# kyleliang919/distributed-lion-pytorch

Hardware: AMD Instinct MI355X
Metric: tokens/sec + all-reduce bytes/step, GPT-2 CLM at 1/2/4/8 MI355X (higher is better)
Workload: dtype bf16; 1 GPU; model=gpt2 (124.4M params), trainable_params=124439808, base_weights=bf16, global_batch=160, task=clm, gradient_checkpointing=False, micro_batch=20, grad_accum=8, seq_len=1024, parallelism=dp1, optimizer=distributed Lion (majority vote), lr 0.0001, wd 0.1, exchange=a2a, impl=native

## Files before the change

distributed_lion_pytorch_amd/csrc/bindings.cpp:

```cpp
#include <ATen/ATen.h>
#include <c10/core/DeviceGuard.h>
#include <c10/hip/HIPStream.h>
#include <torch/library.h>

#include <hip/hip_runtime.h>

#include <cmath>
#include <cstdlib>
#include <string>
#include <tuple>
#include <vector>

#include "kernels.h"

namespace dlion {
enum class Layout : int { NT = 0, NN = 1, TN = 2, TT = 3 };
bool lt_gemm(const void* a, int64_t lda, const void* b, int64_t ldb, void* c, int64_t ldc, const void* bias,
             int64_t M, int64_t N, int64_t K, int epi, int device, hipStream_t s, Layout lay, bool accumulate);
}

namespace {

using at::Tensor;

// ... 981 lines not shown
    check_bf16_contig(*dwte, "dwte");
    TORCH_CHECK(dwte->dim() == 2 && dwte->size(1) == C, "dlion embed: dwte must be [V, C]");
    TORCH_CHECK(sid.has_value() && perm.has_value() && sid->numel() == n && perm->numel() == n &&
                    sid->scalar_type() == at::kLong && perm->scalar_type() == at::kLong && sid->is_contiguous() &&
                    perm->is_contiguous(),
                "dlion embed: the token gradient needs sorted ids and their permutation (int64 [n])");
    V = dwte->size(0);
  }
  if (dwpe.has_value()) {
    check_bf16_contig(*dwpe, "dwpe");
    TORCH_CHECK(dwpe->size(-1) == C && dwpe->size(0) >= T, "dlion embed: dwpe must be [>= T, C]");
  }
  const c10::DeviceGuard g(dx.device());
  const auto dp = drop_params(p);
  check_hip(dlion::launch_embed_bwd(dx.data_ptr(), dwte.has_value() ? sid->data_ptr<int64_t>() : nullptr,
                                    dwte.has_value() ? perm->data_ptr<int64_t>() : nullptr,
                                    dwte.has_value() ? dwte->data_ptr() : nullptr,
                                    dwpe.has_value() ? dwpe->data_ptr() : nullptr, n, static_cast<int>(C),
                                    static_cast<int>(T), V, pos_accumulate ? 1 : 0, static_cast<uint32_t>(seed),
                                    dp.first, dp.second, cur_stream()),
            "embed_bwd");
}

void scale_acc_(const Tensor& x, const Tensor& s, const Tensor& y, bool accumulate) {
  check_bf16_contig(x, "x");
  check_bf16_contig(y, "y");
  check_dev(s, "s");
  TORCH_CHECK(s.scalar_type() == at::kFloat && s.numel() >= 1, "dlion scale_acc: s must be float32");
  TORCH_CHECK(x.numel() == y.numel() && x.numel() % 8 == 0, "dlion scale_acc: size mismatch / numel % 8 != 0");
  const c10::DeviceGuard g(x.device());
  check_hip(dlion::launch_scale_acc(x.data_ptr(), s.data_ptr<float>(), y.data_ptr(), x.numel(), accumulate ? 1 : 0,
                                    cur_stream()),
            "scale_acc");
}

Tensor gemm_nt_stamped(const Tensor& a, const Tensor& b, const Tensor& stamps) {
  check_gemm_operand(a, "a");
  check_gemm_operand(b, "b");
  TORCH_CHECK(gemm_nt_supported(a, b), "dlion gemm: unsupported shape");
  const int64_t blocks = ((a.size(0) + 255) / 256) * ((b.size(0) + 255) / 256);
  TORCH_CHECK(stamps.is_cuda() && stamps.scalar_type() == at::kLong && stamps.is_contiguous() &&
                  stamps.numel() >= blocks * 8,
              "dlion gemm: stamps must be int64 [blocks, 8]");
  auto c = at::empty({a.size(0), b.size(0)}, a.options());
  const c10::DeviceGuard g(a.device());
  check_hip(dlion::launch_gemm_nt_stamped(a.data_ptr(), static_cast<int>(a.stride(0)), b.data_ptr(),
                                          static_cast<int>(b.stride(0)), c.data_ptr(), static_cast<int>(c.stride(0)),
                                          static_cast<int>(a.size(0)), static_cast<int>(b.size(0)),
                                          static_cast<int>(a.size(1)),
                                          reinterpret_cast<unsigned long long*>(stamps.data_ptr<int64_t>()),
                                          cur_stream()),
            "gemm_nt_stamped");
  return c;
}

std::tuple<Tensor, Tensor> gemm_nt_gelu_d(const Tensor& a, const Tensor& b, const Tensor& bias, bool exact) {
  auto h = at::empty({a.size(0), b.size(0)}, a.options());
  auto d = at::empty({a.size(0), b.size(0)}, a.options());
  gemm_nt_launch(a, b, h, &bias, &d, exact ? 7 : 6);
  return {h, d};
}

std::tuple<Tensor, Tensor> gemm_nt_dmul(const Tensor& a, const Tensor& b, const Tensor& d) {
  auto dz = at::empty({a.size(0), b.size(0)}, a.options());
  auto part = at::empty({2 * ((a.size(0) + 255) / 256), b.size(0)}, a.options().dtype(at::kFloat));
  gemm_nt_launch(a, b, dz, nullptr, &d, 8, &part);
// ... 358 lines not shown
  Tensor part = check_skinny("skinny_gemm_w4", x, N, bias, out, splits, per);
  const int64_t M = x.size(0);
  check_hip(dlion::launch_skinny_gemm_w4(x.data_ptr(), M == 1 ? K : x.stride(0), qweight.data_ptr<uint8_t>(),
                                         absmax.data_ptr<float>(), code.data_ptr<float>(),
                                         bias.has_value() ? bias->data_ptr() : nullptr, out.data_ptr(),
                                         M == 1 ? N : out.stride(0), part.defined() ? part.data_ptr<float>() : nullptr,
                                         static_cast<int>(M), static_cast<int>(N), static_cast<int>(K),
                                         static_cast<int>(splits), static_cast<int>(per), cur_stream()),
            "skinny_gemm_w4");
}
}

TORCH_LIBRARY(dlion, m) {
  m.def("skinny_gemm_nt(Tensor x, Tensor w, Tensor? bias, Tensor(a!) out, int splits, int per) -> ()");
  m.def("skinny_gemm_w4(Tensor x, Tensor qweight, Tensor absmax, Tensor code, int N, Tensor? bias, Tensor(a!) out,"
        " int splits, int per) -> ()");
  m.def("dequant4_t_(Tensor q, Tensor absmax, Tensor code, Tensor(a!) out) -> ()");
  m.def("transpose_pad(Tensor x, int rows_out=-1) -> Tensor");
  m.def("kv_append(Tensor q, Tensor k, Tensor v, Tensor pos, Tensor? cos, Tensor? sin, Tensor? q_gamma, Tensor? k_gamma,"
        " float eps, Tensor(a!) k_cache, Tensor(b!) v_cache, Tensor(c!) err) -> Tensor");
  m.def("decode_attention(Tensor q, Tensor k_cache, Tensor v_cache, Tensor kv_len, int window, int max_len, int splits,"
        " int chunk) -> Tensor");
  m.def("quant4(Tensor w, Tensor code) -> (Tensor, Tensor)");
  m.def("dequant4_(Tensor q, Tensor absmax, Tensor code, Tensor(a!) out) -> ()");
  m.def("gemm_tn(Tensor[] P, Tensor[] Q, int splits) -> Tensor");
  m.def("gemm_tn_(Tensor[] P, Tensor[] Q, Tensor(a!) out, bool accumulate) -> ()");
  m.def("lora_rows(Tensor x, Tensor w, float scale, float p, int seed) -> Tensor");
  m.def("lora_up(Tensor o, Tensor u, Tensor b, float s) -> Tensor");
  m.def("lora_cols(Tensor g, Tensor y, Tensor? a, float yscale, float p, int seed) -> (Tensor, Tensor)");
  m.def("gemm_nt_dgelu(Tensor a, Tensor b, Tensor bias, Tensor z, bool exact) -> (Tensor, Tensor)");
  m.def("gemm_nt_gelu_d(Tensor a, Tensor b, Tensor bias, bool exact) -> (Tensor, Tensor)");
  m.def("gemm_nt_dmul(Tensor a, Tensor b, Tensor d) -> (Tensor, Tensor)");
  m.def("gemm_nt_stamped(Tensor a, Tensor b, Tensor(a!) stamps) -> Tensor");
  m.def("embed_fwd(Tensor ids, Tensor wte, Tensor wpe, float p, int seed, Tensor(a!)? err=None) -> Tensor");
  m.def("index_check_(Tensor ids, int hi, int ignore, Tensor(a!) err, int code) -> ()");
  m.def(
      "embed_bwd_(Tensor dx, Tensor? sid, Tensor? perm, Tensor(a!)? dwte, Tensor(b!)? dwpe, int T, bool pos_accumulate,"
      " float p, int seed) -> ()");
  m.def("scale_acc_(Tensor x, Tensor s, Tensor(a!) y, bool accumulate) -> ()");
  m.def("lt_gemm_nt(Tensor a, Tensor b, Tensor? bias, int epi, Tensor(a!) out) -> bool");
  m.def("lt_gemm_nn(Tensor a, Tensor b, Tensor(a!) out) -> bool");
  m.def("lt_gemm_tn(Tensor a, Tensor b, Tensor(a!) out, bool accumulate) -> bool");
  m.def("lt_gemm_nt_acc(Tensor a, Tensor b, Tensor(a!) out, bool accumulate) -> bool");
  m.def("lt_gemm_layout(Tensor a, Tensor b, Tensor(a!) out, int layout, bool accumulate) -> bool");
  m.def("gemm_nt(Tensor a, Tensor b, Tensor? bias) -> Tensor");
  m.def("gemm_nt_out(Tensor a, Tensor b, Tensor? bias, Tensor(a!) out) -> ()");
  m.def("gemm_nt_gelu(Tensor a, Tensor b, Tensor bias, bool exact) -> (Tensor, Tensor)");
  m.def("swiglu_fwd(Tensor g, Tensor u) -> Tensor");
  m.def("swiglu_bwd(Tensor dh, Tensor g, Tensor u) -> (Tensor, Tensor)");
  m.def("swiglu_bwd_fused(Tensor dh, Tensor g, Tensor u) -> Tensor");
  m.def("swiglu_bwd_fused_t(Tensor dh, Tensor g, Tensor u) -> (Tensor, Tensor)");
  m.def("swiglu_fwd_t(Tensor g, Tensor u) -> (Tensor, Tensor)");
  m.def("rope(Tensor x, Tensor cos, Tensor sin, bool inverse) -> Tensor");
  m.def("rope_(Tensor(a!) x, Tensor cos, Tensor sin, bool inverse) -> ()");
  m.def("qk_norm_rope_fwd(Tensor x, Tensor gamma_a, Tensor? gamma_b, int split, float eps, Tensor cos, Tensor sin)"
        " -> (Tensor, Tensor)");
  m.def("qk_norm_rope_bwd_(Tensor(a!) g, Tensor x, Tensor rstd, Tensor gamma_a, Tensor? gamma_b, int split,"
        " Tensor? cos, Tensor? sin, int parts) -> Tensor");
  m.def(
      "add_norm_fwd(Tensor x, Tensor? y, Tensor? bias, Tensor gamma, Tensor? beta, float eps, bool rms, float p,"
      " int seed) -> (Tensor, Tensor, Tensor, Tensor)");
  m.def(
      "add_norm_bwd(Tensor dh, Tensor? dxo_in, Tensor xo, Tensor gamma, Tensor mean, Tensor rstd, bool rms,"
      " float p, int seed, bool want_dy, int parts) -> (Tensor, Tensor, Tensor)");
  m.def("bias_gelu_fwd(Tensor z, Tensor b, bool exact) -> Tensor");
  m.def("bias_gelu_bwd(Tensor dh, Tensor z, Tensor b, bool exact, int parts) -> (Tensor, Tensor)");
// ... 41 lines not shown
  m.impl("grad_sumsq", &grad_sumsq);
  m.impl("clip_coef", &clip_coef);
  m.impl("softmax_xent_", &softmax_xent_);
  m.impl("softmax_xent_opts_", &softmax_xent_opts_);
  m.impl("lm_score", &lm_score);
  m.impl("lm_topk", &lm_topk);
  m.impl("attn_fwd", &attn_fwd);
  m.impl("attn_bwd", &attn_bwd);
  m.impl("add_norm_fwd", &add_norm_fwd);
  m.impl("add_norm_bwd", &add_norm_bwd);
  m.impl("bias_gelu_fwd", &bias_gelu_fwd);
  m.impl("bias_gelu_bwd", &bias_gelu_bwd);
  m.impl("sum_partials", &sum_partials);
  m.impl("sum_partials_acc_", &sum_partials_acc_);
  m.impl("sum_partials_scaled_", &sum_partials_scaled_);
  m.impl("sum_partials_multi_", &sum_partials_multi_);
  m.impl("colsum_partials", &colsum_partials);
  m.impl("swiglu_fwd", &swiglu_fwd);
  m.impl("swiglu_bwd", &swiglu_bwd);
  m.impl("swiglu_bwd_fused", &swiglu_bwd_fused);
  m.impl("swiglu_bwd_fused_t", &swiglu_bwd_fused_t);
  m.impl("swiglu_fwd_t", &swiglu_fwd_t);
  m.impl("rope", &rope);
  m.impl("rope_", &rope_);
  m.impl("qk_norm_rope_fwd", &qk_norm_rope_fwd);
  m.impl("qk_norm_rope_bwd_", &qk_norm_rope_bwd_);
  m.impl("gemm_nt", &gemm_nt);
  m.impl("gemm_nt_out", &gemm_nt_out);
  m.impl("gemm_nt_gelu", &gemm_nt_gelu);
  m.impl("gemm_nt_dgelu", &gemm_nt_dgelu);
  m.impl("gemm_nt_gelu_d", &gemm_nt_gelu_d);
  m.impl("gemm_nt_dmul", &gemm_nt_dmul);
  m.impl("gemm_nt_stamped", &gemm_nt_stamped);
  m.impl("embed_fwd", &embed_fwd);
  m.impl("index_check_", &index_check_);
  m.impl("embed_bwd_", &embed_bwd_);
  m.impl("scale_acc_", &scale_acc_);
  m.impl("lt_gemm_nt", &lt_gemm_nt);
  m.impl("lt_gemm_nn", &lt_gemm_nn);
  m.impl("lt_gemm_tn", &lt_gemm_tn);
  m.impl("lt_gemm_nt_acc", &lt_gemm_nt_acc);
  m.impl("lt_gemm_layout", &lt_gemm_layout);
  m.impl("gemm_tn", &gemm_tn);
  m.impl("gemm_tn_", &gemm_tn_);
  m.impl("lora_rows", &lora_rows);
  m.impl("lora_up", &lora_up);
  m.impl("lora_cols", &lora_cols);
  m.impl("quant4", &quant4);
  m.impl("dequant4_", &dequant4_);
  m.impl("dequant4_t_", &dequant4_t_);
  m.impl("transpose_pad", &transpose_pad);
  m.impl("kv_append", &kv_append);
  m.impl("decode_attention", &decode_attention);
  m.impl("skinny_gemm_nt", &skinny_gemm_nt);
  m.impl("skinny_gemm_w4", &skinny_gemm_w4);
}
```

distributed_lion_pytorch_amd/csrc/gemm.hip:

```cpp
#include "common.h"

#include <algorithm>

namespace dlion {

namespace {

typedef __bf16 bf16x8 __attribute__((ext_vector_type(8)));
typedef float f32x4 __attribute__((ext_vector_type(4)));

constexpr int kBM = 256, kBN = 256, kBK = 64;
constexpr int kHalf = 128 * kBK * 2;
constexpr int kLds = 8 * kHalf;

struct GemmArgs {
  const uint16_t* A;
  const uint16_t* B;
  uint16_t* C;
  const uint16_t* bias;
  uint16_t* aux;
  float* part;
  unsigned long long* stamps;
  int lda, ldb, ldc, ldaux;
  int M, N, K;
  int tiles_m, tiles_n;
};

__device__ __forceinline__ constexpr int slot(int dbuf, int ab, int half) { return ((dbuf * 2 + ab) * 2 + half) * kHalf; }

__device__ __forceinline__ void vm_wait6() { asm volatile("s_waitcnt vmcnt(6)" ::: "memory"); }
__device__ __forceinline__ void vm_wait8() { asm volatile("s_waitcnt vmcnt(8)" ::: "memory"); }
__device__ __forceinline__ void vm_wait2() { asm volatile("s_waitcnt vmcnt(2)" ::: "memory"); }
__device__ __forceinline__ void vm_wait0() { asm volatile("s_waitcnt vmcnt(0)" ::: "memory"); }

__device__ __forceinline__ void glds16(const uint16_t* base, uint32_t boff, uint8_t* dst) {
  const uint8_t* src = reinterpret_cast<const uint8_t*>(base) + boff;
  __builtin_amdgcn_global_load_lds((const __attribute__((address_space(1))) void*)src,
                                   (__attribute__((address_space(3))) void*)dst, 16, 0, 0);
}

typedef unsigned int u32x4 __attribute__((ext_vector_type(4)));
template <bool NT, typename V>
__device__ __forceinline__ void st16(uint16_t* p, const V& v) {
  const u32x4 x = __builtin_bit_cast(u32x4, v);
  if constexpr (NT) __builtin_nontemporal_store(x, reinterpret_cast<u32x4*>(p));
  else *reinterpret_cast<u32x4*>(p) = x;
}
template <bool NT>
__device__ __forceinline__ uint4 ld16(const uint16_t* p) {
  u32x4 x;
  if constexpr (NT) x = __builtin_nontemporal_load(reinterpret_cast<const u32x4*>(p));
  else x = *reinterpret_cast<const u32x4*>(p);
  return make_uint4(x[0], x[1], x[2], x[3]);
}
constexpr bool kNtAux = true, kNtC = true;
// ... 191 lines not shown
  float bv[4][4] = {};
  if constexpr (EPI == 1) {
#pragma unroll
    for (int nt = 0; nt < 4; ++nt)
#pragma unroll
      for (int j = 0; j < 4; ++j) {
        const int n = n0 + wc * 64 + nt * 16 + 4 * (lane >> 4) + j;
        bv[nt][j] = n < g.N ? bf16_to_f32(g.bias[n]) : 0.f;
      }
  }
  const int row_base = m0 + wr * 128;
  const int col_base = n0 + wc * 64;

  auto park = [&](auto fn) {
#pragma unroll
    for (int mt = 0; mt < 8; ++mt)
#pragma unroll
      for (int nt = 0; nt < 4; ++nt) {
        const int row = mt * 16 + (lane & 15);
        const int col = nt * 16 + 4 * (lane >> 4);
        const int chunk = (col >> 3) ^ (row & 7);
        const uint32_t lo = static_cast<uint32_t>(fn(acc[mt][nt][0], nt, 0)) |
                            (static_cast<uint32_t>(fn(acc[mt][nt][1], nt, 1)) << 16);
        const uint32_t hi = static_cast<uint32_t>(fn(acc[mt][nt][2], nt, 2)) |
                            (static_cast<uint32_t>(fn(acc[mt][nt][3], nt, 3)) << 16);
        *reinterpret_cast<uint2*>(reg + row * 128 + chunk * 16 + (col & 7) * 2) = make_uint2(lo, hi);
      }
    asm volatile("s_waitcnt lgkmcnt(0)" ::: "memory");
    __builtin_amdgcn_wave_barrier();
  };
  const int ch = lane & 7;
  const int gn = col_base + ch * 8;

  if constexpr (EPI <= 1) {
    park([&](float v, int nt, int j) { return __builtin_bit_cast(uint16_t, static_cast<__bf16>(v + bv[nt][j])); });
    DLION_STAMP(st_[3])
#pragma unroll
    for (int i = 0; i < 16; ++i) {
      const int row = i * 8 + (lane >> 3);
      const uint4 v = *reinterpret_cast<const uint4*>(reg + row * 128 + ((ch ^ (row & 7)) << 4));
      const int gm = row_base + row;
      if (gm < g.M && gn < g.N) st16<false>(g.C + (int64_t)gm * g.ldc + gn, v);
    }
    if constexpr (STAMP) {
      DLION_STAMP(st_[4])
      DLION_RSTAMP(st_[6])
      if (tid < 8) g.stamps[static_cast<int64_t>(blockIdx.x) * 8 + tid] = tid < 7 ? st_[tid < 7 ? tid : 0] : 0ull;
    }
  } else if constexpr (EPI <= 3 || EPI == 6 || EPI == 7) {
    park([&](float v, int, int) { return __builtin_bit_cast(uint16_t, static_cast<__bf16>(v)); });
    float b8[8];
    if (gn < g.N) {
      Elem<kBF16>::load8(g.bias + gn, b8);
    } else {
#pragma unroll
      for (int j = 0; j < 8; ++j) b8[j] = 0.f;
    }
#pragma unroll 4
    for (int i = 0; i < 16; ++i) {
      const int row = i * 8 + (lane >> 3);
      const uint4 v = *reinterpret_cast<const uint4*>(reg + row * 128 + ((ch ^ (row & 7)) << 4));
      const int gm = row_base + row;
      if (gm < g.M && gn < g.N) {
        float z[8];
        Elem<kBF16>::load8(reinterpret_cast<const uint16_t*>(&v), z);
        bf16x8 hb;
        if constexpr (EPI <= 3) {
// ... 61 lines not shown
      cs[j] += __shfl_xor(cs[j], 32);
    }
    if (lane < 8 && gn < g.N) {
      float* dst = g.part + (int64_t)(2 * tm + wr) * g.N + gn;
      *reinterpret_cast<float4*>(dst) = make_float4(cs[0], cs[1], cs[2], cs[3]);
      *reinterpret_cast<float4*>(dst + 4) = make_float4(cs[4], cs[5], cs[6], cs[7]);
    }
  }
}

}

hipError_t launch_gemm_nt_stamped(const void* A, int lda, const void* B, int ldb, void* C, int ldc, int M, int N, int K,
                                  unsigned long long* stamps, hipStream_t st) {
  if (K % 128 != 0 || N % 8 != 0) return hipErrorInvalidValue;
  GemmArgs g{};
  g.A = static_cast<const uint16_t*>(A);
  g.B = static_cast<const uint16_t*>(B);
  g.C = static_cast<uint16_t*>(C);
  g.lda = lda;
  g.ldb = ldb;
  g.ldc = ldc;
  g.M = M;
  g.N = N;
  g.K = K;
  g.tiles_m = (M + kBM - 1) / kBM;
  g.tiles_n = (N + kBN - 1) / kBN;
  g.stamps = stamps;
  hipLaunchKernelGGL((gemm_nt_kernel<0, true>), dim3(g.tiles_m * g.tiles_n), dim3(512), 0, st, g);
  return hipGetLastError();
}


hipError_t launch_gemm_nt(const void* A, int lda, const void* B, int ldb, void* C, int ldc, const void* bias,
                          void* aux, int ldaux, int M, int N, int K, int epi, float* part, hipStream_t st) {
  if (M <= 0 || N <= 0) return hipSuccess;
  if (K % 128 != 0 || N % 8 != 0 || lda % 8 != 0 || ldb % 8 != 0 || ldc % 8 != 0) return hipErrorInvalidValue;
  if ((int64_t)M * lda >= (1ll << 31) || (int64_t)N * ldb >= (1ll << 31)) return hipErrorInvalidValue;
  if (epi >= 2 && (aux == nullptr || ldaux % 8 != 0)) return hipErrorInvalidValue;
  if (epi >= 1 && epi != 8 && (bias == nullptr || reinterpret_cast<uintptr_t>(bias) % 16 != 0))
    return hipErrorInvalidValue;
  if ((epi == 4 || epi == 5 || epi == 8) && (part == nullptr || reinterpret_cast<uintptr_t>(part) % 16 != 0))
    return hipErrorInvalidValue;
  GemmArgs g;
  g.A = static_cast<const uint16_t*>(A);
  g.B = static_cast<const uint16_t*>(B);
  g.C = static_cast<uint16_t*>(C);
  g.bias = static_cast<const uint16_t*>(bias);
  g.aux = static_cast<uint16_t*>(aux);
  g.part = part;
  g.lda = lda;
  g.ldb = ldb;
  g.ldc = ldc;
  g.ldaux = ldaux;
  g.M = M;
  g.N = N;
  g.K = K;
  g.tiles_m = (M + kBM - 1) / kBM;
  g.tiles_n = (N + kBN - 1) / kBN;
  const dim3 grid(g.tiles_m * g.tiles_n), block(512);
  switch (epi) {
    case 0: hipLaunchKernelGGL(gemm_nt_kernel<0>, grid, block, 0, st, g); break;
    case 1: hipLaunchKernelGGL(gemm_nt_kernel<1>, grid, block, 0, st, g); break;
    case 2: hipLaunchKernelGGL(gemm_nt_kernel<2>, grid, block, 0, st, g); break;
    case 3: hipLaunchKernelGGL(gemm_nt_kernel<3>, grid, block, 0, st, g); break;
    case 4: hipLaunchKernelGGL(gemm_nt_kernel<4>, grid, block, 0, st, g); break;
    case 5: hipLaunchKernelGGL(gemm_nt_kernel<5>, grid, block, 0, st, g); break;
    case 6: hipLaunchKernelGGL(gemm_nt_kernel<6>, grid, block, 0, st, g); break;
    case 7: hipLaunchKernelGGL(gemm_nt_kernel<7>, grid, block, 0, st, g); break;
    case 8: hipLaunchKernelGGL(gemm_nt_kernel<8>, grid, block, 0, st, g); break;
    default: return hipErrorInvalidValue;
  }
  return hipGetLastError();
}

}
```

distributed_lion_pytorch_amd/csrc/kernels.h:

```cpp
#pragma once
#include <hip/hip_runtime.h>
#include <stdint.h>

#include "attention.h"

namespace dlion {

hipError_t launch_lion_local(int dt, const int64_t* seg, const int64_t* chunks, int64_t n_chunks, float decay,
                             float neg_lr, float b1, float omb1, float b2, float omb2, const float* gscale,
                             hipStream_t st, int rounding = 0, uint32_t rkey = 0, int64_t cbase = 0);
hipError_t launch_lion_encode(int dt, const int64_t* seg, const int64_t* chunks, int64_t n_chunks, uint8_t* bits,
                              float b1, float omb1, float b2, float omb2, int update_m, int stochastic, float rr,
                              uint64_t seed, uint32_t step, const float* gscale, hipStream_t st,
                              int64_t cbase = 0);
hipError_t launch_grad_sumsq(int dt, const int64_t* seg, const int64_t* chunks, int64_t n_chunks, float* partial,
                             hipStream_t st);
hipError_t launch_clip_coef(const float* partial, int64_t n, float max_norm, float* out, hipStream_t st);
hipError_t launch_lion_vote_apply(int dt, const int64_t* seg, const int64_t* chunks, int64_t n_chunks,
                                  const uint8_t* planes, int64_t plane_stride, const uint8_t* alive, int world,
                                  int mode, int tie, const uint8_t* neg, float decay, float neg_lr, const uint8_t* own,
                                  unsigned long long* agree, hipStream_t st, int rounding = 0, uint32_t rkey = 0,
                                  int64_t cbase = 0);
hipError_t launch_vote_reduce(const uint8_t* recv, int64_t nbytes, const uint8_t* alive, int world, int tie,
                              uint8_t* out, uint8_t* neg_out, unsigned long long* ties, hipStream_t st);
// ... 15 lines not shown
hipError_t launch_bias_gelu_bwd(const void* dh, const void* z, const void* b, void* dz, float* dbpart, int parts,
                                int64_t rows, int N, bool exact, hipStream_t st);
hipError_t launch_swiglu_fwd(const void* g, const void* u, void* h, int64_t rows, int64_t F, int64_t ld_in,
                             hipStream_t st);
hipError_t launch_swiglu_fwd_t(const void* g, const void* u, void* h, void* ht, int64_t rows, int64_t F,
                               int64_t ld_in, hipStream_t st);
hipError_t launch_swiglu_bwd_t(const void* dh, const void* g, const void* u, void* dgu, void* dgut, int64_t rows,
                               int64_t F, int64_t ld_in, hipStream_t st);
hipError_t launch_swiglu_bwd(const void* dh, const void* g, const void* u, void* dg, void* du, int64_t rows,
                             int64_t F, int64_t ld_in, int64_t ld_out, hipStream_t st);
hipError_t launch_rope(const void* x, const void* cos, const void* sin, void* y, int64_t rows, int T, int H, int D,
                       bool inverse, int64_t x_ld, int64_t y_ld, hipStream_t st);
hipError_t launch_qk_norm_rope_fwd(const void* x, const void* gamma_a, const void* gamma_b, const void* cos,
                                   const void* sin, void* y, float* rstd, int64_t rows, int T, int Hx, int D,
                                   int split, float eps, int64_t x_ld, hipStream_t st);
hipError_t launch_qk_norm_rope_bwd(void* g, const void* x, const float* rstd, const void* gamma_a, const void* gamma_b,
                                   const void* cos, const void* sin, float* part, int parts, int64_t rows, int T,
                                   int Hx, int D, int split, int64_t g_ld, int64_t x_ld, hipStream_t st);
hipError_t launch_sum_partials(const float* part, int S, int64_t n, int64_t ld, void* out, bool accumulate,
                               hipStream_t st, const float* scale = nullptr);
hipError_t launch_colsum(const void* x, float* part, int parts, int64_t rows, int N, hipStream_t st);
hipError_t launch_sum_partials_multi(const float* const* ptrs, const int64_t* rows, const int64_t* lds, int nseg,
                                     int64_t n, void* out, bool accumulate, hipStream_t st);
int sum_partials_split_factor(int64_t n, int64_t total_rows);
hipError_t launch_transpose_pad(const void* x, int64_t R, int64_t C, int64_t ldx, void* out, int64_t Rp,
                                hipStream_t st);
hipError_t launch_sum_partials_split(const float* const* ptrs, const int64_t* rows, const int64_t* lds, int nseg,
                                     int64_t n, int Y, float* scratch, void* out, bool accumulate, const float* scale,
                                     hipStream_t st);

hipError_t launch_gemm_nt(const void* A, int lda, const void* B, int ldb, void* C, int ldc, const void* bias,
                          void* aux, int ldaux, int M, int N, int K, int epi, float* part, hipStream_t st);

hipError_t launch_embed_fwd(const int64_t* ids, const void* wte, const void* wpe, void* out, int64_t n, int C, int T,
                            int64_t V, uint32_t seed, uint32_t thresh16, float inv_keep, int32_t* err, hipStream_t st);
constexpr int kIndexErrEmbed = 1, kIndexErrLabel = 2, kIndexErrCache = 8;
hipError_t launch_index_check(const int64_t* ids, int64_t n, int64_t hi, int64_t ignore, int32_t* err, int code,
                              hipStream_t st);
hipError_t launch_embed_bwd(const void* dx, const int64_t* sid, const int64_t* perm, void* dwte, void* dwpe, int64_t n,
                            int C, int T, int64_t V, int pos_accumulate, uint32_t seed, uint32_t thresh16,
                            float inv_keep, hipStream_t st);
hipError_t launch_scale_acc(const void* x, const float* s, void* y, int64_t n, int accumulate, hipStream_t st);

hipError_t launch_gemm_tn(const void* const* P, const void* const* Q, int nseg, int64_t seg_rows, int ldp, int ldq,
                          float* C, int M, int N, int splits, bool accumulate, hipStream_t st, void* Cb = nullptr);

hipError_t launch_gemm_nt_stamped(const void* A, int lda, const void* B, int ldb, void* C, int ldc, int M, int N, int K,
                                  unsigned long long* stamps, hipStream_t st);

hipError_t launch_lora_rows(const void* in, int64_t ldin, const void* w, void* out, int64_t rows, int K, int r,
                            float scale, uint32_t seed, uint32_t thresh16, float inv_keep, hipStream_t st);
hipError_t launch_lora_up(const void* o, int64_t ldo, const void* u, const void* b, void* out, int64_t rows, int N, int r,
                          float s, hipStream_t st);
int lora_cols_parts(int64_t rows, int N);
hipError_t launch_lora_cols(const void* g, int64_t ldg, const void* y, const void* a, void* dx, float* part, int64_t rows,
                            int N, int r, int parts, int mode, float yscale, uint32_t seed, uint32_t thresh16,
                            float inv_keep, hipStream_t st);
bool lora_wide_rank(int r);
hipError_t launch_lora_rows_wide(const void* in, int64_t ldin, const void* w, void* out, int64_t rows, int K, int r,
                                 float scale, uint32_t seed, uint32_t thresh16, float inv_keep, hipStream_t st);
hipError_t launch_lora_up_wide(const void* o, int64_t ldo, const void* u, const void* b, void* out, int64_t rows, int N,
                               int r, float s, hipStream_t st);
int lora_cols_parts_wide(int64_t rows, int N, int r);
hipError_t launch_lora_cols_wide(const void* g, int64_t ldg, const void* y, const void* a, void* dx, float* part,
                                 int64_t rows, int N, int r, int parts, int mode, float yscale, uint32_t seed,
                                 uint32_t thresh16, float inv_keep, hipStream_t st);
// ... 40 lines not shown
```

distributed_lion_pytorch_amd/ops/fused.py:

```python
from __future__ import annotations

import contextlib
from typing import NamedTuple

import torch
import torch.nn.functional as F

from . import hip
from .linear import _Fn, gemm_fwd

_IMPL = {"mode": "auto"}


def set_impl(mode: str) -> None:
    if mode not in ("auto", "torch", "hip"):
        raise ValueError(mode)
    _IMPL["mode"] = mode


def get_impl() -> str:
    return _IMPL["mode"]


def _use_hip(t: torch.Tensor) -> bool:
    mode = _IMPL["mode"]
    if mode == "torch" or not t.is_cuda:
        return False
    if mode == "hip" or not hip.fallback_allowed():
        hip.require()
        return True
    return hip.available()


def layer_norm(x: torch.Tensor, ln: torch.nn.LayerNorm) -> torch.Tensor:
    return F.layer_norm(x, ln.normalized_shape, ln.weight, ln.bias, ln.eps)
# ... 427 lines not shown
        if ctx.needs_input_grad[0]:
            grads[0] = gemm_fwd(dz, w_fc)
        for i, (w, a, g) in ((1, (ctx.wparams[0], x, dz)), (3, (ctx.wparams[1], h, dy))):
            if ctx.needs_input_grad[i]:
                if ctx.fuse[(i - 1) // 2]:
                    wgrad_into(a, g, w)
                else:
                    grads[i] = wgrad(a, g)
        if ctx.needs_input_grad[2]:
            if ctx.fused_b is not None:
                deposit_grad(ctx.fused_b, part)
            else:
                grads[2] = _sum_rows(part)
        return tuple(grads)


def mlp_gelu(x: torch.Tensor, w_fc: torch.Tensor, b_fc: torch.Tensor, w_proj: torch.Tensor,
             exact: bool = False) -> torch.Tensor:
    shp = x.shape[:-1] + (w_proj.shape[1],)
    x2 = x.reshape(-1, x.shape[-1])
    if x2.is_cuda and _use_hip(x2):
        from .linear import autocast_inputs

        x2, w_fc, b_fc, w_proj = autocast_inputs(x2, w_fc, b_fc, w_proj)
        if (x2.dtype == w_fc.dtype == b_fc.dtype == w_proj.dtype == torch.bfloat16 and w_fc.shape[1] % 8 == 0
                and b_fc.is_contiguous() and w_fc.is_contiguous() and w_proj.is_contiguous()):
            with torch.autocast("cuda", enabled=False):
                return _MLP.apply(x2.contiguous(), w_fc, b_fc, w_proj, bool(exact)).view(shp)
    h = F.gelu(x2 @ w_fc + b_fc, approximate="none" if exact else "tanh")
    return (h @ w_proj).view(shp)


_IDX_EMBED, _IDX_LABEL, _IDX_POS, _IDX_CACHE = 1, 2, 4, 8
_IDX_FLAGS: dict = {}


def _index_flag(dev: torch.device) -> torch.Tensor:
    st = _IDX_FLAGS.get(dev)
    if st is None:
        st = _IDX_FLAGS[dev] = [torch.zeros(1, dtype=torch.int32, device=dev),
                                torch.zeros(1, dtype=torch.int32).pin_memory(), None]
    return st[0]


def _index_error(code: int, where: str):
    msgs = []
    if code & _IDX_EMBED:
        msgs.append("a token id is outside the embedding table [0, vocab_size) -- is the tokenizer larger than "
                    "the model vocabulary? (run_clm resizes the embeddings for that)")
    if code & _IDX_LABEL:
        msgs.append("a label is outside [0, vocab_size) and is not the ignore index -100")
    if code & _IDX_POS:
        msgs.append(_POS_MSG)
    if code & _IDX_CACHE:
        msgs.append("a decode step's position is outside the KV cache [0, max_len) -- the cache is shorter than "
                    "prompt + new tokens")
    return ValueError(f"dlion ({where}): " + "; ".join(msgs))


def check_labels(labels1d: torch.Tensor, v: int) -> None:
    if labels1d.is_cuda and hip.available():
        hip.ops().index_check_(labels1d.contiguous(), int(v), -100, _index_flag(labels1d.device), _IDX_LABEL)
    elif not labels1d.is_cuda:
        bad = ((labels1d < 0) & (labels1d != -100)) | (labels1d >= v)
        if bool(bad.any()):
            raise _index_error(_IDX_LABEL, "labels")


def check_index_errors(blocking: bool = False) -> None:
    for dev, st in _IDX_FLAGS.items():
        flag, host, ev = st
        if blocking:
            code = int(flag.item())
        else:
            code = 0
            if ev is not None:
                if not ev.query():
                    continue
                code = int(host[0])
            host.copy_(flag, non_blocking=True)
            st[2] = torch.cuda.Event()
            st[2].record()
        if code:
            flag.zero_()
            st[2] = None
            raise _index_error(code, str(dev))


class _Embed(torch.autograd.Function):
# ... 896 lines not shown
        lv = logits[:, : ctx.v]
        w = ctx.weight
        if w is not None and w.grad is not None and w.grad.is_contiguous() and w.grad.dtype == torch.bfloat16:
            ops.gemm_tn_([lv], [hs], w.grad, True)
        else:
            out = torch.empty(ctx.v, h2d.shape[1], dtype=torch.bfloat16, device=h2d.device)
            ops.gemm_tn_([lv], [hs], out, False)
            if w is not None:
                w.grad = out if w.grad is None else w.grad + out
            else:
                gw = out
        return gh, gw, None, None, None, None


def _lm_late_ok(weight, logits, h2d, v) -> bool:
    from . import linear

    if not (logits.is_cuda and weight.dtype == torch.bfloat16 and v % 8 == 0
            and hip.available()):
        return False
    lv = logits[:, :v]
    return (linear._tn_eligible(lv, h2d)
            and linear.tn_split_factor(logits.shape[0], v, h2d.shape[1], direct=True) == 1)


def _lm_defer_ok(weight, logits, h2d) -> bool:
    from . import linear

    return (_LM_DEFER and logits.is_cuda and linear._WDEFER_ON and linear._ST.fuse["on"]
            and linear._ST.fuse["multi"] and not linear._ST.fuse["nodefer"] and linear._fuse_target(weight)
            and logits.shape[1] % 8 == 0 and linear._tn_eligible(logits, h2d) and hip.available())




def _softmax_xent_torch_(logits: torch.Tensor, labels: torch.Tensor, v: int, label_smoothing: float = 0.0,
                         z_loss: float = 0.0) -> torch.Tensor:
    x = logits[:, :v].float()
    lse = torch.logsumexp(x, dim=1)
    valid = labels != -100
    safe = labels.clamp_min(0)
    tgt = x.gather(1, safe[:, None]).squeeze(1)
    if label_smoothing != 0.0 or z_loss != 0.0:
        eps, z = float(label_smoothing), float(z_loss)
        row = lse - (1.0 - eps) * tgt - eps * x.mean(dim=1) + z * lse * lse
        row_loss = torch.where(valid, row, torch.zeros_like(lse))
        prob = torch.exp(x - lse[:, None]) * (1.0 + 2.0 * z * lse)[:, None] - eps / v
        prob.scatter_add_(1, safe[:, None], torch.full_like(tgt, -(1.0 - eps))[:, None])
        prob[~valid] = 0.0
        logits[:, :v] = prob.to(logits.dtype)
        if logits.shape[1] > v:
            logits[:, v:] = 0
        return row_loss
    row_loss = torch.where(valid, lse - tgt, torch.zeros_like(lse))
    prob = torch.exp(x - lse[:, None])
    prob.scatter_add_(1, safe[:, None], -torch.ones_like(tgt)[:, None])
    prob[~valid] = 0.0
    logits[:, :v] = prob.to(logits.dtype)
    if logits.shape[1] > v:
        logits[:, v:] = 0
    return row_loss


class _TokenLogp(_Fn):

    @staticmethod
# ... 23 lines not shown

def token_logps(h: torch.Tensor, weight: torch.Tensor, labels: torch.Tensor) -> torch.Tensor:
    h2d = h.reshape(-1, h.shape[-1])
    lab = labels.reshape(-1)
    if h2d.is_cuda:
        from .linear import autocast_inputs

        h2d, weight = autocast_inputs(h2d.contiguous(), weight)
        with torch.autocast("cuda", enabled=False):
            return _TokenLogp.apply(h2d, weight, lab).view(labels.shape)
    if h2d.dtype != weight.dtype:
        h2d = h2d.to(weight.dtype)
    return _TokenLogp.apply(h2d.contiguous(), weight, lab).view(labels.shape)


def check_loss_options(label_smoothing: float, z_loss: float):
    eps, z = float(label_smoothing), float(z_loss)
    if not 0.0 <= eps < 1.0:
        raise ValueError(f"label_smoothing must be in [0, 1), got {label_smoothing!r}")
    if not z >= 0.0 or z == float("inf"):
        raise ValueError(f"z_loss must be a finite value >= 0, got {z_loss!r}")
    return eps, z


def lm_head_cross_entropy(h: torch.Tensor, weight: torch.Tensor, labels: torch.Tensor,
                          normalizer=None, label_smoothing: float = 0.0, z_loss: float = 0.0) -> torch.Tensor:
    eps, z = check_loss_options(label_smoothing, z_loss)
    h2d = h.reshape(-1, h.shape[-1])
    if h2d.is_cuda:
        from .linear import autocast_inputs

        h2d, weight = autocast_inputs(h2d, weight)
        with torch.autocast("cuda", enabled=False):
            return _LMHeadCE.apply(h2d, weight, labels.reshape(-1), normalizer, eps, z)
    if h2d.dtype != weight.dtype:
        h2d = h2d.to(weight.dtype)
    return _LMHeadCE.apply(h2d, weight, labels.reshape(-1), normalizer, eps, z)


def shift_labels(labels: torch.Tensor) -> torch.Tensor:
    out = torch.full_like(labels, -100)
    out[..., :-1] = labels[..., 1:]
    return out


def causal_lm_loss(h: torch.Tensor, weight: torch.Tensor, labels: torch.Tensor, normalizer=None,
                   label_smoothing: float = 0.0, z_loss: float = 0.0) -> torch.Tensor:
    return lm_head_cross_entropy(h, weight, shift_labels(labels), normalizer=normalizer,
                                 label_smoothing=label_smoothing, z_loss=z_loss)


class LMScore(NamedTuple):

    loss: torch.Tensor
    row_loss: torch.Tensor
    lse: torch.Tensor
    pred: torch.Tensor
    rank: torch.Tensor


_SCORE_DTYPES = (torch.float32, torch.bfloat16, torch.float16)


def _lm_score_torch(logits: torch.Tensor, labels: torch.Tensor, v: int, label_smoothing: float = 0.0,
                    z_loss: float = 0.0):
    x = logits[:, :v].float()
# ... 116 lines not shown
```

Before: 1.108 million tokens/s.

## Fuse LM-head softmax into GEMM epilogue via exp relative to label logit

Adds a cross-entropy path for the LM head. A small kernel first computes each row's label logit. The GEMM epilogue then writes exp(logit - label logit) directly in bf16, together with per-tile row partial sums, so no separate softmax pass over the logits is needed. A finish kernel reduces the partials into the loss and a per-row scale. The input gradient is computed in forward with a row-scaled GEMM, and the weight gradient reuses the unnormalised exponentials with row-scaled activations. This path is on by default for large vocabularies; rows whose exponent exceeds the clamp are flagged, which trades some numerical range for the removed passes over the logits.

Measured after the change: 1.054 million tokens/s. 4.8% lower.

```diff
diff --git a/distributed_lion_pytorch_amd/csrc/bindings.cpp b/distributed_lion_pytorch_amd/csrc/bindings.cpp
--- a/distributed_lion_pytorch_amd/csrc/bindings.cpp
+++ b/distributed_lion_pytorch_amd/csrc/bindings.cpp
@@ -1037,6 +1037,77 @@
   check_hip(dlion::launch_scale_acc(x.data_ptr(), s.data_ptr<float>(), y.data_ptr(), x.numel(), accumulate ? 1 : 0,
                                     cur_stream()),
             "scale_acc");
+}
+
+void check_f32_vec(const Tensor& t, int64_t n, const char* name) {
+  TORCH_CHECK(t.is_cuda() && t.scalar_type() == at::kFloat && t.is_contiguous() && t.numel() >= n,
+              "dlion lm_expref: ", name, " must be a contiguous fp32 GPU tensor of >= ", n, " elements");
+}
+
+std::tuple<Tensor, Tensor, Tensor, Tensor> lm_expref_fwd(const Tensor& h, const Tensor& wp, const Tensor& labels,
+                                                         int64_t v, const Tensor& n_valid, const Tensor& err,
+                                                         int64_t code) {
+  check_gemm_operand(h, "h");
+  check_gemm_operand(wp, "wp");
+  TORCH_CHECK(gemm_nt_supported(h, wp), "dlion lm_expref: unsupported shape h=", h.sizes(), " wp=", wp.sizes(),
+              " (needs C % 128 == 0, Vp % 8 == 0)");
+  const int64_t M = h.size(0), C = h.size(1), Vp = wp.size(0);
+  TORCH_CHECK(labels.is_cuda() && labels.scalar_type() == at::kLong && labels.is_contiguous() && labels.numel() == M,
+              "dlion lm_expref: labels must be contiguous int64 [M]");
+  TORCH_CHECK(v > 0 && v <= Vp, "dlion lm_expref: need 0 < v <= Vp");
+  check_f32_vec(n_valid, 1, "n_valid");
+  const c10::DeviceGuard g(h.device());
+  const int64_t P = 4 * ((Vp + 255) / 256);
+  auto fopt = h.options().dtype(at::kFloat);
+  auto q = at::empty({M, Vp}, h.options());
+  auto zpart = at::empty({P, M}, fopt);
+  auto ref = at::empty({M}, fopt), loss = at::empty({M}, fopt), s = at::empty({M}, fopt);
+  int32_t* ep = err_ptr(err, h);
+  check_hip(dlion::launch_lm_ref(h.data_ptr(), h.stride(0), wp.data_ptr(), wp.stride(0), labels.data_ptr<int64_t>(), M,
+                                 static_cast<int>(C), static_cast<int>(v), ref.data_ptr<float>(), cur_stream()),
+            "lm_ref");
+  check_hip(dlion::launch_gemm_nt_rows(h.data_ptr(), static_cast<int>(h.stride(0)), wp.data_ptr(),
+                                       static_cast<int>(wp.stride(0)), q.data_ptr(), static_cast<int>(Vp),
+                                       static_cast<int>(M), static_cast<int>(Vp), static_cast<int>(C), 9,
+                                       ref.data_ptr<float>(), zpart.data_ptr<float>(), static_cast<int>(v), ep,
+                                       static_cast<int>(code), cur_stream()),
+            "gemm_nt (exp - ref)");
+  check_hip(dlion::launch_lm_finish(zpart.data_ptr<float>(), static_cast<int>(P), M, labels.data_ptr<int64_t>(),
+                                    static_cast<int>(v), n_valid.data_ptr<float>(), q.data_ptr(), Vp,
+                                    loss.data_ptr<float>(), s.data_ptr<float>(), ep, static_cast<int>(code),
+                                    cur_stream()),
+            "lm_finish");
+  return {q, zpart, loss, s};
+}
+
+Tensor gemm_nt_rowscale(const Tensor& a, const Tensor& b, const Tensor& s) {
+  check_gemm_operand(a, "a");
+  check_gemm_operand(b, "b");
+  TORCH_CHECK(gemm_nt_supported(a, b), "dlion gemm: unsupported shape a=", a.sizes(), " b=", b.sizes(),
+              " (needs K % 128 == 0, N % 8 == 0)");
+  check_f32_vec(s, a.size(0), "s");
+  const c10::DeviceGuard g(a.device());
+  auto c = at::empty({a.size(0), b.size(0)}, a.options());
+  check_hip(dlion::launch_gemm_nt_rows(a.data_ptr(), static_cast<int>(a.stride(0)), b.data_ptr(),
+                                       static_cast<int>(b.stride(0)), c.data_ptr(), static_cast<int>(c.stride(0)),
+                                       static_cast<int>(a.size(0)), static_cast<int>(b.size(0)),
+                                       static_cast<int>(a.size(1)), 10, s.data_ptr<float>(), nullptr, 0, nullptr, 0,
+                                       cur_stream()),
+            "gemm_nt (row scale)");
+  return c;
+}
+
+Tensor lm_rowscale(const Tensor& x, const Tensor& s, const Tensor& gs) {
+  check_gemm_operand(x, "x");
+  check_f32_vec(s, x.size(0), "s");
+  check_f32_vec(gs, 1, "g");
+  TORCH_CHECK(x.size(1) % 8 == 0, "dlion lm_rowscale: C % 8 != 0");
+  const c10::DeviceGuard g(x.device());
+  auto out = at::empty({x.size(0), x.size(1)}, x.options());
+  check_hip(dlion::launch_lm_rowscale(x.data_ptr(), x.stride(0), s.data_ptr<float>(), gs.data_ptr<float>(),
+                                      out.data_ptr(), x.size(0), static_cast<int>(x.size(1)), cur_stream()),
+            "lm_rowscale");
+  return out;
 }
 
 Tensor gemm_nt_stamped(const Tensor& a, const Tensor& b, const Tensor& stamps) {
@@ -1461,6 +1532,10 @@
   m.def("gemm_nt_gelu_d(Tensor a, Tensor b, Tensor bias, bool exact) -> (Tensor, Tensor)");
   m.def("gemm_nt_dmul(Tensor a, Tensor b, Tensor d) -> (Tensor, Tensor)");
   m.def("gemm_nt_stamped(Tensor a, Tensor b, Tensor(a!) stamps) -> Tensor");
+  m.def("lm_expref_fwd(Tensor h, Tensor wp, Tensor labels, int v, Tensor n_valid, Tensor(a!) err, int code)"
+        " -> (Tensor, Tensor, Tensor, Tensor)");
+  m.def("gemm_nt_rowscale(Tensor a, Tensor b, Tensor s) -> Tensor");
+  m.def("lm_rowscale(Tensor x, Tensor s, Tensor g) -> Tensor");
   m.def("embed_fwd(Tensor ids, Tensor wte, Tensor wpe, float p, int seed, Tensor(a!)? err=None) -> Tensor");
   m.def("index_check_(Tensor ids, int hi, int ignore, Tensor(a!) err, int code) -> ()");
   m.def(
@@ -1568,6 +1643,9 @@
   m.impl("gemm_nt_gelu_d", &gemm_nt_gelu_d);
   m.impl("gemm_nt_dmul", &gemm_nt_dmul);
   m.impl("gemm_nt_stamped", &gemm_nt_stamped);
+  m.impl("lm_expref_fwd", &lm_expref_fwd);
+  m.impl("gemm_nt_rowscale", &gemm_nt_rowscale);
+  m.impl("lm_rowscale", &lm_rowscale);
   m.impl("embed_fwd", &embed_fwd);
   m.impl("index_check_", &index_check_);
   m.impl("embed_bwd_", &embed_bwd_);
diff --git a/distributed_lion_pytorch_amd/csrc/gemm.hip b/distributed_lion_pytorch_amd/csrc/gemm.hip
--- a/distributed_lion_pytorch_amd/csrc/gemm.hip
+++ b/distributed_lion_pytorch_amd/csrc/gemm.hip
@@ -21,6 +21,10 @@
   uint16_t* aux;
   float* part;
   unsigned long long* stamps;
+  const float* rowv;
+  int32_t* err;
+  int err_code;
+  int V;
   int lda, ldb, ldc, ldaux;
   int M, N, K;
   int tiles_m, tiles_n;
@@ -278,7 +282,47 @@
   const int ch = lane & 7;
   const int gn = col_base + ch * 8;
 
-  if constexpr (EPI <= 1) {
+  if constexpr (EPI == 10) {
+#pragma unroll
+    for (int mt = 0; mt < 8; ++mt) {
+      const float sv = g.rowv[min(row_base + mt * 16 + (lane & 15), g.M - 1)];
+#pragma unroll
+      for (int nt = 0; nt < 4; ++nt)
+#pragma unroll
+        for (int j = 0; j < 4; ++j) acc[mt][nt][j] = sv == 0.f ? 0.f : sv * acc[mt][nt][j];
+    }
+  }
+  if constexpr (EPI == 9) {
+    float rf[16];
+#pragma unroll
+    for (int i = 0; i < 16; ++i) rf[i] = g.rowv[min(row_base + i * 8 + (lane >> 3), g.M - 1)];
+    park([&](float v, int, int) { return __builtin_bit_cast(uint16_t, static_cast<__bf16>(v)); });
+    bool clamped = false;
+#pragma unroll 4
+    for (int i = 0; i < 16; ++i) {
+      const int row = i * 8 + (lane >> 3);
+      const uint4 v = *reinterpret_cast<const uint4*>(reg + row * 128 + ((ch ^ (row & 7)) << 4));
+      const int gm = row_base + row;
+      float z[8];
+      Elem<kBF16>::load8(reinterpret_cast<const uint16_t*>(&v), z);
+      bf16x8 qb;
+      float rs = 0.f;
+#pragma unroll
+      for (int j = 0; j < 8; ++j) {
+        const bool real = gn + j < g.V;
+        const float a = (z[j] - rf[i]) * kLog2e;
+        clamped |= real && gm < g.M && a > 126.f;
+        qb[j] = static_cast<__bf16>(real ? __builtin_amdgcn_exp2f(fminf(a, 126.f)) : 0.f);
+        rs += static_cast<float>(qb[j]);
+      }
+      if (gm < g.M && gn < g.N) st16<false>(g.C + (int64_t)gm * g.ldc + gn, qb);
+      rs += __shfl_xor(rs, 1);
+      rs += __shfl_xor(rs, 2);
+      rs += __shfl_xor(rs, 4);
+      if (ch == 0 && gm < g.M) g.part[(int64_t)(4 * tn + wc) * g.M + gm] = rs;
+    }
+    if (clamped) atomicOr(g.err, g.err_code);
+  } else if constexpr (EPI <= 1 || EPI == 10) {
     park([&](float v, int nt, int j) { return __builtin_bit_cast(uint16_t, static_cast<__bf16>(v + bv[nt][j])); });
     DLION_STAMP(st_[3])
 #pragma unroll
@@ -406,6 +450,37 @@
 }
 
 
+hipError_t launch_gemm_nt_rows(const void* A, int lda, const void* B, int ldb, void* C, int ldc, int M, int N, int K,
+                               int epi, const float* rowv, float* zpart, int v, int32_t* err, int err_code,
+                               hipStream_t st) {
+  if (M <= 0 || N <= 0) return hipSuccess;
+  if (K % 128 != 0 || N % 8 != 0 || lda % 8 != 0 || ldb % 8 != 0 || ldc % 8 != 0) return hipErrorInvalidValue;
+  if ((int64_t)M * lda >= (1ll << 31) || (int64_t)N * ldb >= (1ll << 31)) return hipErrorInvalidValue;
+  if (rowv == nullptr || (epi != 9 && epi != 10)) return hipErrorInvalidValue;
+  if (epi == 9 && (zpart == nullptr || err == nullptr || v <= 0 || v > N)) return hipErrorInvalidValue;
+  GemmArgs g{};
+  g.A = static_cast<const uint16_t*>(A);
+  g.B = static_cast<const uint16_t*>(B);
+  g.C = static_cast<uint16_t*>(C);
+  g.part = zpart;
+  g.rowv = rowv;
+  g.err = err;
+  g.err_code = err_code;
+  g.V = v;
+  g.lda = lda;
+  g.ldb = ldb;
+  g.ldc = ldc;
+  g.M = M;
+  g.N = N;
+  g.K = K;
+  g.tiles_m = (M + kBM - 1) / kBM;
+  g.tiles_n = (N + kBN - 1) / kBN;
+  const dim3 grid(g.tiles_m * g.tiles_n), block(512);
+  if (epi == 9) hipLaunchKernelGGL(gemm_nt_kernel<9>, grid, block, 0, st, g);
+  else hipLaunchKernelGGL(gemm_nt_kernel<10>, grid, block, 0, st, g);
+  return hipGetLastError();
+}
+
 hipError_t launch_gemm_nt(const void* A, int lda, const void* B, int ldb, void* C, int ldc, const void* bias,
                           void* aux, int ldaux, int M, int N, int K, int epi, float* part, hipStream_t st) {
   if (M <= 0 || N <= 0) return hipSuccess;
@@ -416,7 +491,7 @@
     return hipErrorInvalidValue;
   if ((epi == 4 || epi == 5 || epi == 8) && (part == nullptr || reinterpret_cast<uintptr_t>(part) % 16 != 0))
     return hipErrorInvalidValue;
-  GemmArgs g;
+  GemmArgs g{};
   g.A = static_cast<const uint16_t*>(A);
   g.B = static_cast<const uint16_t*>(B);
   g.C = static_cast<uint16_t*>(C);
diff --git a/distributed_lion_pytorch_amd/csrc/kernels.h b/distributed_lion_pytorch_amd/csrc/kernels.h
--- a/distributed_lion_pytorch_amd/csrc/kernels.h
+++ b/distributed_lion_pytorch_amd/csrc/kernels.h
@@ -71,6 +71,17 @@
 hipError_t launch_gemm_nt(const void* A, int lda, const void* B, int ldb, void* C, int ldc, const void* bias,
                           void* aux, int ldaux, int M, int N, int K, int epi, float* part, hipStream_t st);
 
+hipError_t launch_gemm_nt_rows(const void* A, int lda, const void* B, int ldb, void* C, int ldc, int M, int N, int K,
+                               int epi, const float* rowv, float* zpart, int v, int32_t* err, int err_code,
+                               hipStream_t st);
+
+hipError_t launch_lm_ref(const void* h, int64_t ldh, const void* w, int64_t ldw, const int64_t* labels, int64_t rows,
+                         int C, int V, float* ref, hipStream_t st);
+hipError_t launch_lm_finish(const float* zpart, int P, int64_t rows, const int64_t* labels, int V, const float* n_valid,
+                            void* q, int64_t ldq, float* loss, float* s, int32_t* err, int err_code, hipStream_t st);
+hipError_t launch_lm_rowscale(const void* x, int64_t ldx, const float* s, const float* g, void* out, int64_t rows, int C,
+                              hipStream_t st);
+
 hipError_t launch_embed_fwd(const int64_t* ids, const void* wte, const void* wpe, void* out, int64_t n, int C, int T,
                             int64_t V, uint32_t seed, uint32_t thresh16, float inv_keep, int32_t* err, hipStream_t st);
 constexpr int kIndexErrEmbed = 1, kIndexErrLabel = 2, kIndexErrCache = 8;
diff --git a/distributed_lion_pytorch_amd/csrc/lm_expref.hip b/distributed_lion_pytorch_amd/csrc/lm_expref.hip
--- /dev/null
+++ b/distributed_lion_pytorch_amd/csrc/lm_expref.hip
@@ -0,0 +1,108 @@
+#include "common.h"
+#include "kernels.h"
+
+namespace dlion {
+
+namespace {
+
+__global__ void __launch_bounds__(256) lm_ref_kernel(const uint16_t* __restrict__ h, int64_t ldh,
+                                                     const uint16_t* __restrict__ w, int64_t ldw,
+                                                     const int64_t* __restrict__ labels, int64_t rows, int C, int V,
+                                                     float* __restrict__ ref) {
+  const int lane = threadIdx.x & 63;
+  const int64_t r = static_cast<int64_t>(blockIdx.x) * 4 + (threadIdx.x >> 6);
+  if (r >= rows) return;
+  const int64_t lab = labels[r];
+  const int64_t c = (lab >= 0 && lab < V) ? lab : 0;
+  const uint16_t* hp = h + r * ldh;
+  const uint16_t* wp = w + c * ldw;
+  float acc = 0.f;
+  for (int k = lane * 8; k < C; k += 512) {
+    float a[8], b[8];
+    Elem<kBF16>::load8(hp + k, a);
+    Elem<kBF16>::load8(wp + k, b);
+#pragma unroll
+    for (int j = 0; j < 8; ++j) acc = __builtin_fmaf(a[j], b[j], acc);
+  }
+  acc = wave_sum_dpp(acc);
+  if (lane == 0) ref[r] = acc;
+}
+
+__global__ void __launch_bounds__(512) lm_finish_kernel(const float* __restrict__ zpart, int P, int64_t rows,
+                                                        const int64_t* __restrict__ labels, int V,
+                                                        const float* __restrict__ n_valid, uint16_t* __restrict__ q,
+                                                        int64_t ldq, float* __restrict__ loss, float* __restrict__ s,
+                                                        int32_t* __restrict__ err, int err_code) {
+  __shared__ float part[8][64];
+  const int rl = threadIdx.x & 63, sl = threadIdx.x >> 6;
+  const int64_t r = static_cast<int64_t>(blockIdx.x) * 64 + rl;
+  float z = 0.f;
+  if (r < rows) {
+    const int p0 = static_cast<int>(static_cast<int64_t>(P) * sl / 8), p1 = static_cast<int>(static_cast<int64_t>(P) * (sl + 1) / 8);
+    for (int p = p0; p < p1; ++p) z += zpart[static_cast<int64_t>(p) * rows + r];
+  }
+  part[sl][rl] = z;
+  __syncthreads();
+  if (sl != 0 || r >= rows) return;
+  z = part[0][rl];
+#pragma unroll
+  for (int t = 1; t < 8; ++t) z += part[t][rl];
+  const int64_t lab = labels[r];
+  const bool valid = lab >= 0 && lab < V;
+  loss[r] = valid ? __logf(z) : 0.f;
+  const float sv = valid ? 1.f / (z * fmaxf(n_valid[0], 1.f)) : 0.f;
+  s[r] = sv;
+  if (valid && !(sv > 0.f)) atomicOr(err, err_code);
+  if (valid) {
+    uint16_t* ql = q + r * ldq + lab;
+    *ql = f32_to_bf16(bf16_to_f32(*ql) - z);
+  }
+}
+
+__global__ void __launch_bounds__(256) lm_rowscale_kernel(const uint16_t* __restrict__ x, int64_t ldx,
+                                                          const float* __restrict__ s, const float* __restrict__ g,
+                                                          uint16_t* __restrict__ out, int64_t rows, int C) {
+  const int per_row = C >> 3;
+  const int64_t i = static_cast<int64_t>(blockIdx.x) * 256 + threadIdx.x;
+  if (i >= rows * per_row) return;
+  const int64_t r = i / per_row;
+  const int c = static_cast<int>(i - r * per_row) << 3;
+  const float f = s[r] * g[0];
+  float v[8];
+  Elem<kBF16>::load8(x + r * ldx + c, v);
+#pragma unroll
+  for (int j = 0; j < 8; ++j) v[j] *= f;
+  Elem<kBF16>::store8(out + r * C + c, v);
+}
+
+}
+
+hipError_t launch_lm_ref(const void* h, int64_t ldh, const void* w, int64_t ldw, const int64_t* labels, int64_t rows,
+                         int C, int V, float* ref, hipStream_t st) {
+  if (rows <= 0) return hipSuccess;
+  if (C % 8 != 0 || ldh % 8 != 0 || ldw % 8 != 0 || V <= 0) return hipErrorInvalidValue;
+  hipLaunchKernelGGL(lm_ref_kernel, dim3(static_cast<unsigned>((rows + 3) / 4)), dim3(256), 0, st,
+                     static_cast<const uint16_t*>(h), ldh, static_cast<const uint16_t*>(w), ldw, labels, rows, C, V, ref);
+  return hipGetLastError();
+}
+
+hipError_t launch_lm_finish(const float* zpart, int P, int64_t rows, const int64_t* labels, int V, const float* n_valid,
+                            void* q, int64_t ldq, float* loss, float* s, int32_t* err, int err_code, hipStream_t st) {
+  if (rows <= 0) return hipSuccess;
+  if (P <= 0 || V <= 0 || V > ldq || err == nullptr) return hipErrorInvalidValue;
+  hipLaunchKernelGGL(lm_finish_kernel, dim3(static_cast<unsigned>((rows + 63) / 64)), dim3(512), 0, st, zpart, P, rows,
+                     labels, V, n_valid, static_cast<uint16_t*>(q), ldq, loss, s, err, err_code);
+  return hipGetLastError();
+}
+
+hipError_t launch_lm_rowscale(const void* x, int64_t ldx, const float* s, const float* g, void* out, int64_t rows, int C,
+                              hipStream_t st) {
+  if (rows <= 0) return hipSuccess;
+  if (C % 8 != 0 || ldx % 8 != 0) return hipErrorInvalidValue;
+  const int64_t n = rows * (C / 8);
+  hipLaunchKernelGGL(lm_rowscale_kernel, dim3(static_cast<unsigned>((n + 255) / 256)), dim3(256), 0, st,
+                     static_cast<const uint16_t*>(x), ldx, s, g, static_cast<uint16_t*>(out), rows, C);
+  return hipGetLastError();
+}
+
+}
diff --git a/distributed_lion_pytorch_amd/ops/fused.py b/distributed_lion_pytorch_amd/ops/fused.py
--- a/distributed_lion_pytorch_amd/ops/fused.py
+++ b/distributed_lion_pytorch_amd/ops/fused.py
@@ -1,6 +1,7 @@
 from __future__ import annotations
 
 import contextlib
+import os
 from typing import NamedTuple
 
 import torch
@@ -494,6 +495,7 @@
 
 
 _IDX_EMBED, _IDX_LABEL, _IDX_POS, _IDX_CACHE = 1, 2, 4, 8
+_IDX_LM_CLAMP = 16
 _IDX_FLAGS: dict = {}
 
 
@@ -517,6 +519,10 @@
     if code & _IDX_CACHE:
         msgs.append("a decode step's position is outside the KV cache [0, max_len) -- the cache is shorter than "
                     "prompt + new tokens")
+    if code & _IDX_LM_CLAMP:
+        msgs.append("the LM head met a logit more than 126 ln 2 = 87.3 above its row's label logit, which its "
+                    "exp(logit - label logit) form cannot hold: the loss and the gradients of that step used a "
+                    "clamped value -- set DLION_LM_EXPREF=0 to train with the softmax kernel instead")
     return ValueError(f"dlion ({where}): " + "; ".join(msgs))
 
 
@@ -1479,6 +1485,118 @@
             and logits.shape[1] % 8 == 0 and linear._tn_eligible(logits, h2d) and hip.available())
 
 
+_LM_EXPREF = os.environ.get("DLION_LM_EXPREF", "1")
+_LM_EXPREF_MIN_BYTES = 256 << 20
+
+
+def _lm_pad128(weight: torch.Tensor):
+    from .linear import cached_derived, fast_transpose
+
+    v = weight.shape[0]
+    vp = (v + 127) // 128 * 128
+    if vp == (v + 63) // 64 * 64:
+        wp, tag = _pad_rows(weight), "pad_t"
+    else:
+        def pad(t):
+            return torch.cat([t, t.new_zeros(vp - v, t.shape[1])], 0)
+
+        wp = cached_derived(weight, "pad_rows128", pad) if isinstance(weight, torch.nn.Parameter) else pad(weight.detach())
+        tag = "pad_t128"
+    if isinstance(weight, torch.nn.Parameter):
+        return wp, cached_derived(weight, tag, lambda t: fast_transpose(t, vp))
+    return wp, fast_transpose(weight.detach(), vp)
+
+
+def _lm_expref_ok(h2d: torch.Tensor, weight: torch.Tensor) -> bool:
+    if _LM_EXPREF == "0" or not (h2d.is_cuda and h2d.dtype == weight.dtype == torch.bfloat16 and h2d.dim() == 2
+                                 and weight.dim() == 2 and torch.is_grad_enabled()
+                                 and (h2d.requires_grad or weight.requires_grad) and _use_hip(h2d)):
+        return False
+    m, c = h2d.shape
+    v = weight.shape[0]
+    vp = (v + 127) // 128 * 128
+    if not (c % 128 == 0 and h2d.stride(1) == 1 and h2d.stride(0) % 8 == 0 and h2d.data_ptr() % 16 == 0
+            and weight.is_contiguous() and weight.data_ptr() % 16 == 0 and m > 0
+            and m * max(vp, h2d.stride(0)) < 2 ** 31 and vp * c < 2 ** 31):
+        return False
+    if _LM_EXPREF == "force":
+        return True
+    tiles = -(-m // 256) * -(-c // 256)
+    return isinstance(weight, torch.nn.Parameter) and tiles < 256 and vp >= 8192 and 2 * m * vp >= _LM_EXPREF_MIN_BYTES
+
+
+def lm_expref_model64(h: torch.Tensor, w: torch.Tensor, labels: torch.Tensor, normalizer=None, g: float = 1.0):
+    h64, w64 = h.detach().double(), w.detach().double()
+    valid = labels != -100
+    col = torch.where(valid, labels, torch.zeros_like(labels))
+    logits = h64 @ w64.t()
+    ref = logits.gather(1, col[:, None])
+    q = torch.exp(logits - ref)
+    z = q.sum(1)
+    n = valid.sum().clamp_min(1).double() if normalizer is None else torch.as_tensor(normalizer).double().clamp_min(1)
+    loss = torch.where(valid, torch.log(z), torch.zeros_like(z)).sum() / n
+    s = torch.where(valid, 1.0 / (z * n), torch.zeros_like(z))
+    q.scatter_add_(1, col[:, None], -(z * valid)[:, None])
+    dh = s[:, None] * (q @ w64)
+    dw = q.t() @ ((g * s)[:, None] * h64)
+    return loss, g * dh, dw
+
+
+class _LMHeadExpRef(_Fn):
+
+    @staticmethod
+    def forward(ctx, h2d, weight, labels1d, normalizer=None):
+        v = weight.shape[0]
+        labels1d = labels1d.contiguous()
+        if normalizer is None:
+            n_valid = (labels1d != -100).sum().clamp_min(1).to(torch.float32)
+        else:
+            n_valid = torch.as_tensor(normalizer, dtype=torch.float32, device=h2d.device).clamp_min(1)
+        check_labels(labels1d, v)
+        wp, wpt = _lm_pad128(weight)
+        ops = hip.ops()
+        q, _, row_loss, s = ops.lm_expref_fwd(h2d, wp, labels1d, v, n_valid.reshape(1), _index_flag(h2d.device),
+                                              _IDX_LM_CLAMP)
+        loss = row_loss.sum() / n_valid
+        dh = ops.gemm_nt_rowscale(q, wpt, s) if ctx.needs_input_grad[0] else h2d.new_empty(0)
+        ctx.weight = weight
+        if ctx.needs_input_grad[1]:
+            ctx.defer = _lm_defer_ok(weight, q, h2d)
+            ctx.save_for_backward(dh, q, s, h2d)
+        else:
+            ctx.save_for_backward(dh)
+        return loss
+
+    @staticmethod
+    def backward(ctx, g):
+        from . import linear
+
+        ops = hip.ops()
+        gs = g.float().reshape(1)
+        dh = ctx.saved_tensors[0]
+        gh = gw = None
+        if ctx.needs_input_grad[0]:
+            gh = torch.empty_like(dh)
+            ops.scale_acc_(dh, gs, gh, False)
+        if not ctx.needs_input_grad[1]:
+            return gh, None, None, None
+        _, q, s, h2d = ctx.saved_tensors
+        w = ctx.weight
+        v, c = w.shape
+        hs = ops.lm_rowscale(h2d, s, gs)
+        if not linear._tn_eligible(q, hs):
+            return gh, (q.t() @ hs)[:v], None, None
+        split = linear.tn_split_factor(q.shape[0], q.shape[1], c)
+        if ctx.defer and linear._defer_wgrad([w], [(0, v * c)], q, hs, split):
+            return gh, None, None, None
+        part = ops.gemm_tn([q], [hs], split).view(split, -1)[:, : v * c]
+        if linear._fuse_target(w):
+            linear.deposit_grad(w, part, defer=False)
+        else:
+            gw = linear.sum_partials_into(part).view(v, c)
+        return gh, gw, None, None
+
+
 
 
 def _softmax_xent_torch_(logits: torch.Tensor, labels: torch.Tensor, v: int, label_smoothing: float = 0.0,
@@ -1568,6 +1686,8 @@
 
         h2d, weight = autocast_inputs(h2d, weight)
         with torch.autocast("cuda", enabled=False):
+            if eps == 0.0 and z == 0.0 and _lm_expref_ok(h2d, weight):
+                return _LMHeadExpRef.apply(h2d, weight, labels.reshape(-1), normalizer)
             return _LMHeadCE.apply(h2d, weight, labels.reshape(-1), normalizer, eps, z)
     if h2d.dtype != weight.dtype:
         h2d = h2d.to(weight.dtype)
```
